# WeiZhang1988/YDORBSLAM

Hardware: AMD Instinct MI355X
Metric: ORB extract+match Mkeypoints/sec (higher is better)
Workload: dtype u8

## Files before the change

### ydorbslam_amd/csrc/extract_kernels.hip.h

```cpp
#pragma once
#include <hip/hip_runtime.h>
#include <stdint.h>

#include "quadtree_core.h"
#include "quadtree_flat.h"

#pragma clang fp contract(off)

namespace ydorb {

constexpr int kPad = 19;
constexpr int kBorder = 16;
constexpr int kMaxLevels = 8;
constexpr int kTileMax = 72;
#ifndef QT_THREADS
#define QT_THREADS 512
#endif
constexpr int kQtThreads = QT_THREADS;

struct LevelDev {
  int w, h, pitch;
  int padOff;
  int blurOff, blurPitch;
  int cellBegin, nCells;
  int quota;
  int candOff;
  int kpOff;
  int tabOff;
  int nodeTabOff;
  float scale;
  float size;
};
struct PlanDev {
  int nLevels, nCellsTotal, cellCap, sumQuota;
  int maxX[16];
  unsigned nodeTabFrameStride;
  int blurTileBegin[kMaxLevels + 1];
  int borderBegin[kMaxLevels + 1];
  LevelDev lv[kMaxLevels];
};
#ifndef BLUR_TH
#define BLUR_TH 58
#endif
constexpr int kBlurTW = 64, kBlurTH = BLUR_TH;
struct CellDev {
  short level, x0, y0, x1, y1, pad0;
  int srcOff;
};

__device__ __forceinline__ int reflect101(int i, int n) {
  if (n == 1) return 0;
  while (i < 0 || i >= n) i = i < 0 ? -i : 2 * (n - 1) - i;
  return i;
}

typedef uint32_t __attribute__((aligned(1))) u32_unaligned;
typedef unsigned long long __attribute__((aligned(1))) u64_unaligned;

#ifndef PYR_ROWS
#define PYR_ROWS 8
#endif
constexpr int kPyrRows = PYR_ROWS;
__global__ __launch_bounds__(256) void k_pyr_level0(const uint8_t* __restrict__ img, int stride, size_t frameStride,
                                                    uint8_t* __restrict__ pyr, size_t pyrFrameStride, LevelDev L) {
  const int wx = blockIdx.x * 64 + (threadIdx.x & 63);
  const int yb = (blockIdx.y * 4 + __builtin_amdgcn_readfirstlane(threadIdx.x >> 6)) * kPyrRows;
  const int x0 = wx * 4 - kPad;
  if (x0 + 3 < 0 || x0 >= L.w) return;
  const uint8_t* src = img + (size_t)blockIdx.z * frameStride;
  uint8_t* dst = pyr + (size_t)blockIdx.z * pyrFrameStride + L.padOff + (size_t)kPad * L.pitch + wx * 4;
  const int xa = L.w >= 4 ? min(max(x0, 0), L.w - 4) : 0, sh = 8 * (x0 - xa);
  uint32_t v[kPyrRows];
#pragma unroll
  for (int r = 0; r < kPyrRows; r++) {
    const uint8_t* row = src + (size_t)min(yb + r, L.h - 1) * stride;
    if (L.w >= 4) {
      v[r] = *reinterpret_cast<const u32_unaligned*>(row + xa);
    } else {
      v[r] = 0;
      for (int b = 0; b < L.w; b++) v[r] |= (uint32_t)row[b] << (8 * b);
    }
    v[r] = sh < 0 ? v[r] << (-sh) : v[r] >> sh;
  }
#pragma unroll
  for (int r = 0; r < kPyrRows; r++)
    if (yb + r < L.h) *reinterpret_cast<uint32_t*>(dst + (size_t)(yb + r) * L.pitch) = v[r];
}

__global__ __launch_bounds__(256) void k_pyr_resize(uint8_t* __restrict__ pyr, size_t pyrFrameStride, LevelDev Lp, LevelDev L,
                                                    double scaleX, const short* __restrict__ alpha,
                                                    const int* __restrict__ yofs, const short* __restrict__ beta) {
  const int wx = blockIdx.x * 64 + (threadIdx.x & 63);
  const int yb = (blockIdx.y * 4 + __builtin_amdgcn_readfirstlane(threadIdx.x >> 6)) * kPyrRows;
  const int x0 = wx * 4 - kPad;
  if (x0 + 3 < 0 || x0 >= L.w) return;
  uint8_t* frame = pyr + (size_t)blockIdx.z * pyrFrameStride;
  const uint8_t* S = frame + Lp.padOff + (size_t)kPad * Lp.pitch + kPad;
  uint8_t* dst = frame + L.padOff + (size_t)kPad * L.pitch + wx * 4;
  int sx[4], sx1[4], a0[4], a1[4];
#pragma unroll
  for (int b = 0; b < 4; b++) {
    const int dx = min(max(x0 + b, 0), L.w - 1);
    const float fx = (float)__dsub_rn(__dmul_rn((double)dx + 0.5, scaleX), 0.5);
    sx[b] = min(max((int)floorf(fx), 0), Lp.w - 1);
    a0[b] = alpha[2 * dx]; a1[b] = alpha[2 * dx + 1];
    sx1[b] = min(sx[b] + 1, Lp.w - 1);
  }
  const bool fast = sx[3] - sx[0] <= 6;
  const uint8_t *r0p[kPyrRows], *r1p[kPyrRows];
  int b0[kPyrRows], b1[kPyrRows];
#pragma unroll
  for (int r = 0; r < kPyrRows; r++) {
    const int dy = min(yb + r, L.h - 1);
    const int sy = yofs[dy];
    b0[r] = beta[2 * dy]; b1[r] = beta[2 * dy + 1];
    r0p[r] = S + (size_t)min(max(sy, 0), Lp.h - 1) * Lp.pitch;
    r1p[r] = S + (size_t)min(max(sy + 1, 0), Lp.h - 1) * Lp.pitch;
  }
// ... 1076 lines not shown
  const int c4 = (threadIdx.x & 15) * 4;
#pragma unroll
  for (int r = threadIdx.x >> 4; r < TH; r += 16) {
    const int gy = y0 + r;
    if (!(gy < L.h && x0 + c4 < L.blurPitch)) continue;
    typedef unsigned short u16x2 __attribute__((ext_vector_type(2)));
    const bool odd = r & 1;
    const u16x2 k0 = odd ? u16x2{0, 18} : u16x2{18, 34}, k1 = odd ? u16x2{34, 48} : u16x2{48, 56};
    const u16x2 k2 = odd ? u16x2{56, 48} : u16x2{48, 34}, k3 = odd ? u16x2{34, 18} : u16x2{18, 0};
    const uint32_t* hp = &hb[(r >> 1) * TW + c4];
    const uint4 p0 = *reinterpret_cast<const uint4*>(hp), p1 = *reinterpret_cast<const uint4*>(hp + TW);
    const uint4 p2 = *reinterpret_cast<const uint4*>(hp + 2 * TW), p3 = *reinterpret_cast<const uint4*>(hp + 3 * TW);
    const uint32_t q0[4] = {p0.x, p0.y, p0.z, p0.w}, q1[4] = {p1.x, p1.y, p1.z, p1.w}, q2[4] = {p2.x, p2.y, p2.z, p2.w}, q3[4] = {p3.x, p3.y, p3.z, p3.w};
    uint32_t acc[4];
#pragma unroll
    for (int k = 0; k < 4; k++) {
      acc[k] = __builtin_amdgcn_udot2(__builtin_bit_cast(u16x2, q0[k]), k0, 32768u, false);
      acc[k] = __builtin_amdgcn_udot2(__builtin_bit_cast(u16x2, q1[k]), k1, acc[k], false);
      acc[k] = __builtin_amdgcn_udot2(__builtin_bit_cast(u16x2, q2[k]), k2, acc[k], false);
      acc[k] = __builtin_amdgcn_udot2(__builtin_bit_cast(u16x2, q3[k]), k3, acc[k], false);
    }
    const uint32_t out = (acc[0] >> 16) | ((acc[1] >> 16) << 8) | ((acc[2] >> 16) << 16) | ((acc[3] >> 16) << 24);
    *reinterpret_cast<uint32_t*>(blur + (size_t)f * blurFrameStride + L.blurOff + (size_t)gy * L.blurPitch + x0 + c4) = out;
  }
}

__device__ __forceinline__ float fast_atan2_deg(float y, float x) {
  const float p1 = 0.9997878412794807f * (float)(180 / 3.14159265358979323846);
  const float p3 = -0.3258083974640975f * (float)(180 / 3.14159265358979323846);
  const float p5 = 0.1555786518463281f * (float)(180 / 3.14159265358979323846);
  const float p7 = -0.04432655554792128f * (float)(180 / 3.14159265358979323846);
  const float eps = (float)2.2204460492503131e-16;
  const float ax = fabsf(x), ay = fabsf(y);
  float a, c, c2;
  if (ax >= ay) {
    c = __fdiv_rn(ay, __fadd_rn(ax, eps));
    c2 = __fmul_rn(c, c);
    a = __fmul_rn(__fadd_rn(__fmul_rn(__fadd_rn(__fmul_rn(__fadd_rn(__fmul_rn(p7, c2), p5), c2), p3), c2), p1), c);
  } else {
    c = __fdiv_rn(ax, __fadd_rn(ay, eps));
    c2 = __fmul_rn(c, c);
    a = __fsub_rn(90.f, __fmul_rn(__fadd_rn(__fmul_rn(__fadd_rn(__fmul_rn(__fadd_rn(__fmul_rn(p7, c2), p5), c2), p3), c2), p1), c));
  }
  if (x < 0) a = __fsub_rn(180.f, a);
  if (y < 0) a = __fsub_rn(360.f, a);
  return a;
}

__device__ __forceinline__ void sincos_det(float xf, float* sinOut, float* cosOut) {
  const double x = (double)xf;
  const double n = rint(__dmul_rn(x, 6.36619772367581382433e-01));
  const double r = __dsub_rn(__dsub_rn(x, __dmul_rn(n, 1.57079632673412561417e+00)), __dmul_rn(n, 6.07710050650619224932e-11));
  const double z = __dmul_rn(r, r);
  double p = __dmul_rn(z, 1.58969099521155010221e-10);
  p = __dadd_rn(p, -2.50507602534068634195e-08); p = __dmul_rn(p, z);
  p = __dadd_rn(p, 2.75573137070700676789e-06);  p = __dmul_rn(p, z);
  p = __dadd_rn(p, -1.98412698298579493134e-04); p = __dmul_rn(p, z);
  p = __dadd_rn(p, 8.33333333332248946124e-03);  p = __dmul_rn(p, z);
  p = __dadd_rn(p, -1.66666666666666324348e-01); p = __dmul_rn(p, z);
  p = __dmul_rn(p, r); p = __dadd_rn(p, r);
  double q = __dmul_rn(z, -1.13596475577881948265e-11);
  q = __dadd_rn(q, 2.08757232129817482790e-09);  q = __dmul_rn(q, z);
  q = __dadd_rn(q, -2.75573143513906633035e-07); q = __dmul_rn(q, z);
  q = __dadd_rn(q, 2.48015872894767294178e-05);  q = __dmul_rn(q, z);
  q = __dadd_rn(q, -1.38888888888741095749e-03); q = __dmul_rn(q, z);
  q = __dadd_rn(q, 4.16666666666666019037e-02);  q = __dmul_rn(q, z);
  q = __dmul_rn(q, z);
  double h = __dmul_rn(z, 0.5);
  h = __dsub_rn(h, q);
  h = __dsub_rn(1.0, h);
  const int quad = ((int)n) & 3;
  const double sv = quad == 0 ? p : quad == 1 ? h : quad == 2 ? -p : -h;
  const double cv = quad == 0 ? h : quad == 1 ? -p : quad == 2 ? -h : p;
  *sinOut = (float)sv;
  *cosOut = (float)cv;
}

__device__ __align__(16) const float kPatternDev[1024] = {
#include "orb_pattern_data.inc"
};

struct YdKeyPointDev { float x, y, size, angle, response; int octave, class_id; };

__global__ __launch_bounds__(256) void k_orient_describe(const uint8_t* __restrict__ pyr, size_t pyrFrameStride,
                                                         const uint8_t* __restrict__ blur, size_t blurFrameStride, PlanDev P,
                                                         const uint32_t* __restrict__ lvlKp, const int* __restrict__ lvlCount,
                                                         YdKeyPointDev* __restrict__ kps, uint8_t* __restrict__ desc, int cap,
                                                         int* __restrict__ nOut, float* __restrict__ lvlAngle) {
  const int lane = threadIdx.x & 63;
  int bx = blockIdx.x, f = blockIdx.y;
  if ((f | 7) < (int)gridDim.y) {
    bx = (f & 7) * (gridDim.x >> 3) + (blockIdx.x >> 3);
    f = (f & ~7) | (blockIdx.x & 7);
  }
  const int slot = bx * 4 + __builtin_amdgcn_readfirstlane(threadIdx.x >> 6);
  if (slot >= P.sumQuota) return;
  float4 pat[4];
#pragma unroll
  for (int t = 0; t < 4; t++) pat[t] = reinterpret_cast<const float4*>(kPatternDev)[t * 64 + lane];
  int level = 0;
#pragma unroll
  for (int l = 1; l < kMaxLevels; l++)
    if (l < P.nLevels && slot >= P.lv[l].kpOff) level = l;
  const uint32_t pk = __builtin_amdgcn_readfirstlane(lvlKp[(size_t)f * P.sumQuota + slot]);
  int before = 0, tot = 0, mine = 0;
#pragma unroll
  for (int l = 0; l < kMaxLevels; l++) {
    const int c = l < P.nLevels ? lvlCount[f * kMaxLevels + l] : 0;
    if (l < level) before += c;
    if (l == level) mine = c;
    tot += c;
  }
  if (slot == 0 && lane == 0) nOut[f] = min(tot, cap);
  const LevelDev L = P.lv[level];
  const int k = slot - L.kpOff;
  if (k >= mine) return;
  const int outIdx = before + k;
  if (outIdx >= cap) return;
  const int kx = qt_x(pk) + kBorder, ky = qt_y(pk) + kBorder;
  const uint8_t* roi = pyr + (size_t)f * pyrFrameStride + L.padOff + (size_t)kPad * L.pitch + kPad;
  const uint8_t* org = roi + (ptrdiff_t)(ky - 15) * L.pitch + (kx - 32);
  const int u = lane - 32;
  unsigned narrow = 0;
#pragma unroll
  for (int v = 1; v <= 15; v++) narrow |= (unsigned)(P.maxX[v] == 0) << v;
  int m10 = 0, m01 = 0;
  if (u >= -15 && u <= 15) m10 = u * org[(unsigned)(15 * L.pitch + lane)];
  if (lane >= 1 && lane <= 15 && ((narrow >> lane) & 1u)) {
    const int pos = org[(unsigned)((15 + lane) * L.pitch + 32)], neg = org[(unsigned)((15 - lane) * L.pitch + 32)];
    m01 = lane * (pos - neg);
  }
#pragma unroll
  for (int v = 1; v <= 15; v++) {
    const int d = P.maxX[v];
    if (d > 0 && u >= -d && u <= d) {
      const int pos = org[(unsigned)((15 + v) * L.pitch + lane)], neg = org[(unsigned)((15 - v) * L.pitch + lane)];
      m01 += v * (pos - neg);
      m10 += u * (pos + neg);
    }
  }
#pragma unroll
  for (int o = 32; o >= 1; o >>= 1) {
    m10 += __shfl_xor(m10, o, 64);
    m01 += __shfl_xor(m01, o, 64);
  }
  const float angle = fast_atan2_deg((float)m01, (float)m10);
  const float rad = __fmul_rn(angle, (float)(3.14159265358979323846 / 180.0));
  float sinB, cosA;
  sincos_det(rad, &sinB, &cosA);
  constexpr int kBias = 24;
  const uint8_t* bl = blur + (size_t)f * blurFrameStride + L.blurOff + (ptrdiff_t)(ky - kBias) * L.blurPitch + (kx - kBias);
  unsigned long long words[4];
#pragma unroll
  for (int t = 0; t < 4; t++) {
    const float4 pt = pat[t];
    const int r0 = __float2int_rn(__fadd_rn(__fmul_rn(pt.x, sinB), __fmul_rn(pt.y, cosA)));
    const int c0 = __float2int_rn(__fsub_rn(__fmul_rn(pt.x, cosA), __fmul_rn(pt.y, sinB)));
    const int r1 = __float2int_rn(__fadd_rn(__fmul_rn(pt.z, sinB), __fmul_rn(pt.w, cosA)));
    const int c1 = __float2int_rn(__fsub_rn(__fmul_rn(pt.z, cosA), __fmul_rn(pt.w, sinB)));
    const int t0 = bl[(unsigned)((r0 + kBias) * L.blurPitch + c0 + kBias)], t1 = bl[(unsigned)((r1 + kBias) * L.blurPitch + c1 + kBias)];
    words[t] = __ballot(t0 < t1);
  }
  if (lane < 4) {
    unsigned long long w = lane == 0 ? words[0] : lane == 1 ? words[1] : lane == 2 ? words[2] : words[3];
    reinterpret_cast<unsigned long long*>(desc + ((size_t)f * cap + outIdx) * 32)[lane] = w;
  }
  if (lane == 0) {
    YdKeyPointDev kp;
    kp.x = (float)kx;
    kp.y = (float)ky;
    if (level) { kp.x = __fmul_rn(kp.x, L.scale); kp.y = __fmul_rn(kp.y, L.scale); }
    kp.size = L.size;
    kp.angle = angle;
    kp.response = (float)qt_r(pk);
    kp.octave = level;
    kp.class_id = -1;
    kps[(size_t)f * cap + outIdx] = kp;
    lvlAngle[(size_t)f * P.sumQuota + slot] = angle;
  }
}


template <int KPW>
__global__ __launch_bounds__(256) void k_orient_describe_n(const uint8_t* __restrict__ pyr, size_t pyrFrameStride,
                                                           const uint8_t* __restrict__ blur, size_t blurFrameStride, PlanDev P,
                                                           const uint32_t* __restrict__ lvlKp, const int* __restrict__ lvlCount,
                                                           YdKeyPointDev* __restrict__ kps, uint8_t* __restrict__ desc, int cap,
                                                           int* __restrict__ nOut, float* __restrict__ lvlAngle) {
  const int lane = threadIdx.x & 63;
  int bx = blockIdx.x, f = blockIdx.y;
  if ((f | 7) < (int)gridDim.y) {
    bx = (f & 7) * (gridDim.x >> 3) + (blockIdx.x >> 3);
    f = (f & ~7) | (blockIdx.x & 7);
  }
  const int slot0 = (bx * 4 + __builtin_amdgcn_readfirstlane(threadIdx.x >> 6)) * KPW;
  if (slot0 >= P.sumQuota) return;
  float4 pat[4];
#pragma unroll
  for (int t = 0; t < 4; t++) pat[t] = reinterpret_cast<const float4*>(kPatternDev)[t * 64 + lane];
  int cnt[kMaxLevels], tot = 0;
#pragma unroll
  for (int l = 0; l < kMaxLevels; l++) { cnt[l] = l < P.nLevels ? lvlCount[f * kMaxLevels + l] : 0; tot += cnt[l]; }
  int level[KPW], outIdx[KPW];
  uint32_t pk[KPW];
  bool valid[KPW];
#pragma unroll
  for (int j = 0; j < KPW; j++) {
    const int slot = min(slot0 + j, P.sumQuota - 1);
    level[j] = 0;
#pragma unroll
    for (int l = 1; l < kMaxLevels; l++)
      if (l < P.nLevels && slot >= P.lv[l].kpOff) level[j] = l;
    pk[j] = __builtin_amdgcn_readfirstlane(lvlKp[(size_t)f * P.sumQuota + slot]);
  }
  if (slot0 == 0 && lane == 0) nOut[f] = min(tot, cap);
  bool any = false;
#pragma unroll
  for (int j = 0; j < KPW; j++) {
    int before = 0, mine = 0;
#pragma unroll
    for (int l = 0; l < kMaxLevels; l++) {
      if (l < level[j]) before += cnt[l];
      if (l == level[j]) mine = cnt[l];
    }
    const int k = slot0 + j - P.lv[level[j]].kpOff;
    outIdx[j] = before + k;
    valid[j] = slot0 + j < P.sumQuota && k < mine && outIdx[j] < cap;
    any = any || valid[j];
  }
  if (!any) return;
  int firstValid = 0;
#pragma unroll
  for (int j = KPW - 1; j >= 0; j--) if (valid[j]) firstValid = j;
#pragma unroll
  for (int j = 0; j < KPW; j++)
    if (!valid[j]) {
#pragma unroll
      for (int i = 0; i < KPW; i++) if (i == firstValid) { pk[j] = pk[i]; level[j] = level[i]; }
    }
  int kx[KPW], ky[KPW], pitch[KPW];
  const uint8_t* org[KPW];
#pragma unroll
  for (int j = 0; j < KPW; j++) {
    const LevelDev& L = P.lv[level[j]];
    kx[j] = qt_x(pk[j]) + kBorder; ky[j] = qt_y(pk[j]) + kBorder;
    pitch[j] = L.pitch;
    const uint8_t* roi = pyr + (size_t)f * pyrFrameStride + L.padOff + (size_t)kPad * L.pitch + kPad;
    org[j] = roi + (ptrdiff_t)(ky[j] - 15) * L.pitch + (kx[j] - 32);
  }
  const int u = lane - 32;
  unsigned narrow = 0;
#pragma unroll
  for (int v = 1; v <= 15; v++) narrow |= (unsigned)(P.maxX[v] == 0) << v;
  int m10[KPW], m01[KPW];
#pragma unroll
  for (int j = 0; j < KPW; j++) {
    m10[j] = 0; m01[j] = 0;
    if (u >= -15 && u <= 15) m10[j] = u * org[j][(unsigned)(15 * pitch[j] + lane)];
    if (lane >= 1 && lane <= 15 && ((narrow >> lane) & 1u)) {
      const int pos = org[j][(unsigned)((15 + lane) * pitch[j] + 32)], neg = org[j][(unsigned)((15 - lane) * pitch[j] + 32)];
      m01[j] = lane * (pos - neg);
    }
  }
#pragma unroll
  for (int v = 1; v <= 15; v++) {
    const int d = P.maxX[v];
    if (d > 0 && u >= -d && u <= d) {
#pragma unroll
      for (int j = 0; j < KPW; j++) {
        const int pos = org[j][(unsigned)((15 + v) * pitch[j] + lane)], neg = org[j][(unsigned)((15 - v) * pitch[j] + lane)];
        m01[j] += v * (pos - neg);
        m10[j] += u * (pos + neg);
      }
    }
  }
#pragma unroll
  for (int o = 32; o >= 1; o >>= 1) {
#pragma unroll
    for (int j = 0; j < KPW; j++) {
      m10[j] += __shfl_xor(m10[j], o, 64);
      m01[j] += __shfl_xor(m01[j], o, 64);
    }
  }
  constexpr int kBias = 24;
  float angle[KPW];
  int tA[KPW][4], tB[KPW][4];
#pragma unroll
  for (int j = 0; j < KPW; j++) {
    const LevelDev& L = P.lv[level[j]];
    angle[j] = fast_atan2_deg((float)m01[j], (float)m10[j]);
    const float rad = __fmul_rn(angle[j], (float)(3.14159265358979323846 / 180.0));
    float sinB, cosA;
    sincos_det(rad, &sinB, &cosA);
    const uint8_t* bl = blur + (size_t)f * blurFrameStride + L.blurOff + (ptrdiff_t)(ky[j] - kBias) * L.blurPitch + (kx[j] - kBias);
#pragma unroll
    for (int t = 0; t < 4; t++) {
      const float4 pt = pat[t];
      const int r0 = __float2int_rn(__fadd_rn(__fmul_rn(pt.x, sinB), __fmul_rn(pt.y, cosA)));
      const int c0 = __float2int_rn(__fsub_rn(__fmul_rn(pt.x, cosA), __fmul_rn(pt.y, sinB)));
      const int r1 = __float2int_rn(__fadd_rn(__fmul_rn(pt.z, sinB), __fmul_rn(pt.w, cosA)));
      const int c1 = __float2int_rn(__fsub_rn(__fmul_rn(pt.z, cosA), __fmul_rn(pt.w, sinB)));
      tA[j][t] = bl[(unsigned)((r0 + kBias) * L.blurPitch + c0 + kBias)];
      tB[j][t] = bl[(unsigned)((r1 + kBias) * L.blurPitch + c1 + kBias)];
    }
  }
#pragma unroll
  for (int j = 0; j < KPW; j++) {
    unsigned long long words[4];
#pragma unroll
    for (int t = 0; t < 4; t++) words[t] = __ballot(tA[j][t] < tB[j][t]);
    if (!valid[j]) continue;
    const LevelDev& L = P.lv[level[j]];
    if (lane < 4) {
      unsigned long long w = lane == 0 ? words[0] : lane == 1 ? words[1] : lane == 2 ? words[2] : words[3];
      reinterpret_cast<unsigned long long*>(desc + ((size_t)f * cap + outIdx[j]) * 32)[lane] = w;
    }
    if (lane == 0) {
      YdKeyPointDev kp;
      kp.x = (float)kx[j];
      kp.y = (float)ky[j];
      if (level[j]) { kp.x = __fmul_rn(kp.x, L.scale); kp.y = __fmul_rn(kp.y, L.scale); }
      kp.size = L.size;
      kp.angle = angle[j];
      kp.response = (float)qt_r(pk[j]);
      kp.octave = level[j];
      kp.class_id = -1;
      kps[(size_t)f * cap + outIdx[j]] = kp;
      lvlAngle[(size_t)f * P.sumQuota + slot0 + j] = angle[j];
    }
  }
}

}
```

### ydorbslam_amd/csrc/orb_extractor.hip

```cpp
#include <hip/hip_runtime.h>
#include <cstdlib>

#include <algorithm>
#include <cmath>
#include <cstdarg>
#include <cstdio>
#include <cstring>
#include <string>
#include <vector>

#include "../../include/ydorb/c_api.h"
#include "extract_kernels.hip.h"
#include "host_buffers.h"
#include "ydorb_host.h"

using namespace ydorb;

namespace {

inline int cvRoundF(float v) { return (int)lrintf(v); }
inline int cvFloorF(float v) { int i = (int)v; return i - (i > v); }
inline int alignUp(int v, int a) { return (v + a - 1) / a * a; }
inline size_t alignUpZ(size_t v, size_t a) { return (v + a - 1) / a * a; }

// ... 92 lines not shown

void buildFusedLevel(HostPlan& P, int l) {
  const PlanDev& D = P.dev;
  const LevelDev& L = D.lv[l];
  HostPlan::FusedLevel& F = P.fused[l];
  F.on = false;
  if (L.w < 20 || L.h < 20) return;
  const int nd = (L.w + 2 * kPad + 3) >> 2;
  auto srcOf = [&](int p) { return p < kPad ? 2 * kPad - p : p < kPad + L.w ? -1 : p < L.w + 2 * kPad ? 2 * L.w + 2 * kPad - 2 - p : -2; };
  int shift = -1;
  for (int sft = 0; sft < 64 && shift < 0; sft++) {
    bool ok = true;
    for (int c = 0; c < nd && ok; c++)
      for (int j = 0; j < 4; j++) {
        const int sp = srcOf(4 * c + j);
        if (sp >= 0 && ((sp >> 2) + sft) >> 6 != (c + sft) >> 6) ok = false;
      }
    if (ok) shift = sft;
  }
  if (shift < 0) return;
  std::vector<PyrColEntry> col;
  if (l > 0) {
    const LevelDev& Lp = D.lv[l - 1];
    const int* xofs = P.tabInt.data() + P.tab[l].xofs;
    const short* alpha = P.tabShort.data() + P.tab[l].alpha;
    col.resize(nd);
    for (int c = 0; c < nd; c++) {
      const int dx0 = std::min(std::max(4 * c - kPad, 0), L.w - 1);
      for (int b = 0; b < 4; b++) {
        const int dx = std::min(std::max(4 * c - kPad + b, 0), L.w - 1);
        const int off = xofs[dx] - xofs[dx0];
        if (off < 0 || off > 6 || xofs[dx0] + 7 >= Lp.w + kPad) return;
        col[c].sel[b] = (uint32_t)off | 0x0c000c00u | ((uint32_t)(off + 1) << 16);
        col[c].ab[b] = (uint32_t)(uint16_t)alpha[2 * dx] | ((uint32_t)(uint16_t)alpha[2 * dx + 1] << 16);
      }
    }
  }
  F.shift = shift;
  F.padOff = (int)P.padTab.size();
  for (int c = 0; c < nd; c++) {
    int dA = -1, dB = -1;
    for (int j = 0; j < 4; j++) {
      const int sp = srcOf(4 * c + j);
      if (sp < 0) continue;
      const int d = sp >> 2;
      if (dA < 0 || d == dA) dA = d;
      else dB = d;
    }
    PyrPadEntry pe{};
    pe.laneA4 = 4u * (unsigned)(((dA < 0 ? c : dA) + shift) & 63);
    pe.laneB4 = 4u * (unsigned)(((dB < 0 ? c : dB) + shift) & 63);
    pe.selM = 0; pe.selF = 0;
    for (int j = 0; j < 4; j++) {
      const int sp = srcOf(4 * c + j);
      uint32_t m = 0x0c, f;
      if (sp == -1) f = (uint32_t)j;
      else if (sp == -2) f = 0x0c;
      else { m = (uint32_t)(sp & 3) + ((sp >> 2) == dA ? 4u : 0u); f = 4u + (uint32_t)j; }
      pe.selM |= m << (8 * j);
      pe.selF |= f << (8 * j);
    }
    P.padTab.push_back(pe);
  }
  if (l > 0) {
    F.colOff = (int)P.colTab.size();
    P.colTab.insert(P.colTab.end(), col.begin(), col.end());
    F.rowOff = (int)P.rowTab.size();
    const int* yofs = P.tabInt.data() + P.tab[l].yofs;
    const short* beta = P.tabShort.data() + P.tab[l].beta;
    const int rows = alignUp(L.h, 4 * kPyrRowsF);
    for (int y = 0; y < rows; y++) {
      const int dy = std::min(y, L.h - 1);
      P.rowTab.push_back(make_int2(yofs[dy], (int)((uint32_t)(uint16_t)beta[2 * dy] | ((uint32_t)(uint16_t)beta[2 * dy + 1] << 16))));
    }
  }
  F.on = true;
}

int buildPlan(ydorb_extractor* e, int w, int h, HostPlan& P) {
  P = HostPlan();
  P.w = w; P.h = h;
  PlanDev& D = P.dev;
  D.nLevels = e->cfg.n_levels;
  for (int v = 0; v < 16; v++) D.maxX[v] = e->maxX[v];
  size_t padOff = 0, blurOff = 0;
  int kpOff = 0, candOff = 0, maxCellDim = 0;
  for (int l = 0; l < D.nLevels; l++) {
    LevelDev& L = D.lv[l];
    L.w = cvRoundF((float)w * e->isf[l]);
    L.h = cvRoundF((float)h * e->isf[l]);
    if (L.w < 1 || L.h < 1 || L.w > 4000 || L.h > 4000) {
      set_error("level %d size %dx%d out of the supported range (1..4000)", l, L.w, L.h);
      return YDORB_ERR_UNSUPPORTED;
    }
    L.pitch = alignUp(L.w + 2 * kPad, 64);
    L.padOff = (int)padOff;
    padOff += alignUpZ((size_t)(L.h + 2 * kPad) * L.pitch, 256);
    L.blurPitch = alignUp(L.w, 64);
    L.blurOff = (int)blurOff;
    blurOff += alignUpZ((size_t)L.h * L.blurPitch, 256);
    L.quota = e->perLevel[l];
    L.kpOff = kpOff;
    kpOff += L.quota;
    L.scale = e->sf[l];
    L.size = (float)(int)(31 * e->sf[l]);
    L.cellBegin = (int)P.cells.size();
    const int minB = kBorder, maxBX = L.w - kBorder, maxBY = L.h - kBorder;
    const float width = (float)(maxBX - minB), height = (float)(maxBY - minB);
    const int colsNum = (int)(width / 30.0f), rowsNum = (int)(height / 30.0f);
    if (colsNum > 0 && rowsNum > 0) {
      const int cellW = (int)ceilf(width / colsNum), cellH = (int)ceilf(height / rowsNum);
      maxCellDim = std::max(maxCellDim, std::max(cellW, cellH));
      P.levelCellDim[l] = std::max(cellW, cellH);
      for (int i = 0; i < rowsNum; i++) {
        const float iniY = (float)(minB + i * cellH);
        float maxY = iniY + cellH + 6;
        if (iniY >= maxBY - 3) continue;
        if (maxY > maxBY) maxY = (float)maxBY;
        for (int j = 0; j < colsNum; j++) {
          const float iniX = (float)(minB + j * cellW);
          float maxX = iniX + cellW + 6;
          if (iniX >= maxBX - 6) continue;
          if (maxX > maxBX) maxX = (float)maxBX;
          CellDev c{};
          c.level = (short)l;
          c.x0 = (short)iniX; c.y0 = (short)iniY; c.x1 = (short)maxX; c.y1 = (short)maxY;
          c.srcOff = L.padOff + (kPad + c.y0) * L.pitch + kPad + c.x0;
          P.cells.push_back(c);
        }
      }
    }
    L.nCells = (int)P.cells.size() - L.cellBegin;
    if (l > 0) {
      const LevelDev& Lp = D.lv[l - 1];
      const double scale_x = 1. / ((double)L.w / Lp.w), scale_y = 1. / ((double)L.h / Lp.h);
      P.tab[l].xofs = (int)P.tabInt.size();
      P.tab[l].alpha = (int)P.tabShort.size();
      for (int dx = 0; dx < L.w; dx++) {
        float fx = (float)((dx + 0.5) * scale_x - 0.5);
        int sx = cvFloorF(fx);
        fx -= sx;
        if (sx < 0) { fx = 0; sx = 0; }
        if (sx >= Lp.w - 1) { fx = 0; sx = Lp.w - 1; }
        P.tabInt.push_back(sx);
        P.tabShort.push_back((short)cvRoundF((1.f - fx) * 2048));
        P.tabShort.push_back((short)cvRoundF(fx * 2048));
      }
      P.tab[l].yofs = (int)P.tabInt.size();
      P.tab[l].beta = (int)P.tabShort.size();
      for (int dy = 0; dy < L.h; dy++) {
        float fy = (float)((dy + 0.5) * scale_y - 0.5);
        int sy = cvFloorF(fy);
        fy -= sy;
        P.tabInt.push_back(sy);
        P.tabShort.push_back((short)cvRoundF((1.f - fy) * 2048));
        P.tabShort.push_back((short)cvRoundF(fy * 2048));
      }
    }
  }
  if (maxCellDim + 6 > kTileMax) {
    set_error("cell size %d exceeds the FAST tile (%d)", maxCellDim, kTileMax - 6);
    return YDORB_ERR_UNSUPPORTED;
  }
  D.nCellsTotal = (int)P.cells.size();
  P.maxCellDim = maxCellDim;
  D.cellCap = alignUp(std::max(((maxCellDim + 1) / 2) * ((maxCellDim + 1) / 2), 64), 64);
  D.sumQuota = kpOff;
// ... 178 lines not shown
      const int maxT = dim + 6, maxB = dim;
      narrow = maxT <= 44;
      const int pitch = narrow ? 48 : 80;
      fl.tileBytes = alignUp((maxT + 3) * pitch, 16);
      fl.scoreBytes = alignUp((maxB + 2) * (maxB + 2) + 4, 16);
      fl.listBytes = alignUp(2 * maxB * maxB, 16);
      return (size_t)4 * (fl.tileBytes + fl.scoreBytes + fl.listBytes);
    };
    {
      FastLds flAll; bool nAll;
      const size_t dynAll = fastGeom(0, D.nLevels, flAll, nAll);
      if (dynAll > 48 * 1024) {
        HIPCHK(hipFuncSetAttribute(reinterpret_cast<const void*>(k_fast_cells<48>), hipFuncAttributeMaxDynamicSharedMemorySize, (int)dynAll));
        HIPCHK(hipFuncSetAttribute(reinterpret_cast<const void*>(k_fast_cells<80>), hipFuncAttributeMaxDynamicSharedMemorySize, (int)dynAll));
      }
    }
    int l0 = 0;
    for (int g = 0; g < e->fastGroups && l0 < D.nLevels; g++) {
      const int l1 = g == e->fastGroups - 1 ? D.nLevels : l0 + 1;
      const int c0 = D.lv[l0].cellBegin, c1 = D.lv[l1 - 1].cellBegin + D.lv[l1 - 1].nCells;
      if (c1 > c0 && D.nCellsTotal > 0) {
        FastLds fl; bool narrow;
        const size_t dyn = fastGeom(l0, l1, fl, narrow);
        const dim3 grid(((c1 - c0 + 3) / 4 + 7) / 8 * 8, nFrames);
        if (narrow) hipLaunchKernelGGL(k_fast_cells<48>, grid, dim3(256), dyn, s, e->d_pyr, P.pyrFrameStride, D, e->d_cells, c0, c1, thr, fl, e->d_cellCount, e->d_cellCand);
        else hipLaunchKernelGGL(k_fast_cells<80>, grid, dim3(256), dyn, s, e->d_pyr, P.pyrFrameStride, D, e->d_cells, c0, c1, thr, fl, e->d_cellCount, e->d_cellCand);
      }
      HIPCHK(hipEventRecord(e->evFast[l0], s));
      fastEv[l0] = e->evFast[l0];
      grpFirst[nGroups] = l0; grpEnd[nGroups] = l1; nGroups++;
      for (int l = l0 + 1; l < l1; l++) fastEv[l] = e->evFast[l0];
      l0 = l1;
    }
  }
  if (prof) HIPCHK(hipEventRecord(e->ev[2], s));
  HIPCHK(hipEventRecord(e->evFork, s));
  hipLaunchKernelGGL(k_blur, dim3((D.blurTileBegin[D.nLevels] + 7) / 8 * 8, nFrames), dim3(256), 0, s, e->d_pyr, P.pyrFrameStride, e->d_blur,
                     P.blurFrameStride, D);
  if (prof) HIPCHK(hipEventRecord(e->ev[3], s));
  bool anyFast = false;
  for (int g = 0; g < nGroups; g++) {
    const int l0 = grpFirst[g], l1 = grpEnd[g];
    const hipStream_t qs = e->qtInline ? s : e->qtStream[g % kMaxLevels];
    if (!e->qtInline) HIPCHK(hipStreamWaitEvent(qs, fastEv[l0] ? fastEv[l0] : e->evFork, 0));
    int items = 8, qmax = 1, tabLen = 2;
    for (int l = l0; l < l1; l++) {
      items = std::max(items, P.qt[l].items); qmax = std::max(qmax, D.lv[l].quota);
      tabLen = std::max(tabLen, std::max(D.lv[l].w - 2 * kBorder, 0) + std::max(D.lv[l].h - 2 * kBorder, 0) + 2);
    }
    const size_t lds = qt_fast_lds_bytes(qmax, tabLen);
    if (!e->forcePassQuadtree && lds <= 150 * 1024) {
      const dim3 grid(nFrames, l1 - l0);
#define YD_QT_FAST(IT) hipLaunchKernelGGL(k_qt_fast<IT>, grid, dim3(kQfThreads), lds, qs, D, e->d_cellCount, e->d_cellCand, l0, qmax, tabLen, e->d_lvlKp, \
                                          e->d_lvlCount, e->d_needPass, e->d_lvlMaxN, e->d_passList, e->d_passList + 1)
      if (items <= 8) YD_QT_FAST(8);
      else if (items <= 16) YD_QT_FAST(16);
      else YD_QT_FAST(32);
#undef YD_QT_FAST
      anyFast = true;
    } else {
      for (int l = l0; l < l1; l++) {
        const HostPlan::QtLevel& Q = P.qt[l];
        hipLaunchKernelGGL(k_quadtree, dim3(1, nFrames), dim3(kQtThreads), Q.lds, qs, D, e->d_cellCount, e->d_cellCand, e->d_qtCand, e->d_qtNode,
                           P.qtFrameStride, Q.nodeCap, Q.candCap, l, e->d_lvlKp, e->d_lvlCount, e->d_status, e->d_nodeScratch);
      }
    }
    if (!e->qtInline) HIPCHK(hipEventRecord(e->evJoin[g], qs));
  }
  if (!e->qtInline) for (int g = 0; g < nGroups; g++) HIPCHK(hipStreamWaitEvent(s, e->evJoin[g], 0));
  if (anyFast) {
    const int seen = e->h_lvlMaxN[kMaxLevels];
    const int listGrid = std::max(1, std::min({kQtPassWorkgroups, D.nLevels * nFrames, seen + seen / 4}));
    hipLaunchKernelGGL(k_quadtree_list, dim3(listGrid), dim3(kQtListThreads), P.qtPassLds, s, D, e->d_cellCount, e->d_cellCand,
                       e->d_qtCand, e->d_qtNode, P.qtFrameStride, -std::max(P.qtPassNodes, 1), e->d_lvlKp, e->d_lvlCount, e->d_status, e->d_passList,
                       e->d_passList + 1, e->d_nodeScratch, e->d_lvlMaxN + kMaxLevels);
    HIPCHK(hipMemsetAsync(e->d_passList, 0, sizeof(int), s));
  }
  if (prof) HIPCHK(hipEventRecord(e->ev[4], s));
  {
    const int kpw = e->descKpw;
    const dim3 gd(((D.sumQuota + 4 * kpw - 1) / (4 * kpw) + 7) / 8 * 8, nFrames);
#define YD_DESC(K) hipLaunchKernelGGL((k_orient_describe_n<K>), gd, dim3(256), 0, s, e->d_pyr, P.pyrFrameStride, e->d_blur, P.blurFrameStride, D, \
                                         e->d_lvlKp, e->d_lvlCount, d_kps, d_desc, cap, d_nOut, e->d_lvlAngle)
    if (kpw == 1)
      hipLaunchKernelGGL(k_orient_describe, gd, dim3(256), 0, s, e->d_pyr, P.pyrFrameStride, e->d_blur,
                         P.blurFrameStride, D, e->d_lvlKp, e->d_lvlCount, d_kps, d_desc, cap, d_nOut, e->d_lvlAngle);
    else if (kpw == 2) YD_DESC(2);
    else YD_DESC(4);
#undef YD_DESC
  }
  if (prof) { HIPCHK(hipEventRecord(e->ev[5], s)); e->profPending = true; }
  HIPCHK(hipMemcpyAsync(e->h_lvlMaxN, e->d_lvlMaxN, sizeof(int) * (kMaxLevels + 1), hipMemcpyDeviceToHost, s));
  HIPCHK(hipGetLastError());
  e->lastFrames = nFrames;
  e->lastStream = s;
  return YDORB_OK;
}

int checkStatus(ydorb_extractor* e) {
  if (*e->h_status == 1) { set_error("more than 65535 FAST candidates in one pyramid level"); return YDORB_ERR_CAPACITY; }
  if (*e->h_status == 3) { set_error("a pyramid level needs the pass quad-tree kernel (more candidates than LDS slots, or a very deep tree) but its quota is too large for that kernel's LDS node table"); return YDORB_ERR_CAPACITY; }
  if (*e->h_status) { set_error("quad-tree node table overflow (status %d)", *e->h_status); return YDORB_ERR_CAPACITY; }
  return YDORB_OK;
}

void collectProfile(ydorb_extractor* e) {
  if (!e->profiling || !e->profPending) return;
  e->profPending = false;
  for (int i = 0; i < ST_COUNT; i++) {
    float ms = 0;
    if (hipEventElapsedTime(&ms, e->ev[i], e->ev[i + 1]) == hipSuccess) e->stageMs[i] += ms;
  }
  e->stageCalls++;
}

}

int ydorb::extractor_pyramid_view(const ydorb_extractor* e, PyramidView* v) {
  if (!e || !v || !e->planValid || e->lastFrames < 1) { set_error("the extractor holds no pyramid (no call yet)"); return YDORB_ERR_INVALID_ARG; }
  v->device = e->cfg.device; v->nLevels = e->cfg.n_levels; v->frames = e->lastFrames; v->frameStride = (long long)e->plan.pyrFrameStride;
  v->stream = e->stream;
  for (int l = 0; l < e->cfg.n_levels; l++) {
    const LevelDev& L = e->plan.dev.lv[l];
    v->roi[l] = e->d_pyr + L.padOff + (size_t)kPad * L.pitch + kPad;
    v->w[l] = L.w; v->h[l] = L.h; v->pitch[l] = L.pitch;
    v->scale[l] = e->sf[l]; v->invScale[l] = e->isf[l];
    v->quota[l] = e->perLevel[l];
  }
  return YDORB_OK;
}

extern "C" {

int ydorb_extractor_create(const YdExtractorConfig* cfg, ydorb_extractor_t** out) {
  if (!cfg || !out) { set_error("null argument"); return YDORB_ERR_INVALID_ARG; }
  *out = nullptr;
  if (cfg->n_levels < 1 || cfg->n_levels > kMaxLevels || cfg->n_features < 1 || !(cfg->scale_factor > 1.0f)) {
    set_error("unsupported extractor config (n_levels 1..8, n_features >= 1, scale_factor > 1)");
    return YDORB_ERR_INVALID_ARG;
  }
  int rc = ydorb::require_device(cfg->device);
  if (rc) return rc;
  ydorb_extractor* e = new ydorb_extractor();
  e->cfg = *cfg;
  if (const char* v = getenv("YDORB_QT_PASS")) e->forcePassQuadtree = v[0] == '1';
  if (const char* v = getenv("YDORB_PYR_FUSED")) e->noFusedPads = v[0] == '0';
  e->descKpw = cfg->max_batch <= 8 ? 1 : 4;
  if (const char* v = getenv("YDORB_DESC_KPW")) e->descKpw = atoi(v) == 1 ? 1 : atoi(v) == 4 ? 4 : 2;
  e->cfg.min_fast_thr = cfg->ini_fast_thr;
  const int L = cfg->n_levels;
  const float s = cfg->scale_factor;
  int per = (int)round(cfg->n_features * (1 - 1.0 / s) / (1.0 - pow(1.0 / s, L)));
  int sum = 0;
  for (int i = 0; i < L; i++) {
    e->sf.push_back((float)pow(s, i));
    e->sf2.push_back((float)pow(s, 2 * i));
    e->isf.push_back((float)pow(s, -i));
    e->isf2.push_back((float)pow(s, -2 * i));
    if (i < L - 1) {
      e->perLevel.push_back(per);
      sum += per;
      per = (int)round((float)per / s);
    } else {
      e->perLevel.push_back(std::max(cfg->n_features - sum, 0));
    }
  }
  e->sumQuota = 0;
  for (int q : e->perLevel) e->sumQuota += q;
  {
    const int half = 15;
    std::vector<int> mx(half + 1, 0);
    const int maxY = (int)floor(half * sqrt(2.0) / 2.0 + 1.0), minY = (int)ceil(half * sqrt(2.0) / 2.0);
    for (int v = 0; v <= maxY; v++) mx.push_back((int)round(sqrt((double)half * half + (double)v * v)));
    for (int v = half, i = 0; v >= minY; v--) {
      while (mx[i] == mx[i + 1]) i++;
      mx[v] = i;
      i++;
    }
    for (int v = 0; v < 16; v++) e->maxX[v] = mx[v];
  }
  if (hipStreamCreateWithFlags(&e->stream, hipStreamNonBlocking) != hipSuccess) {
    set_error("hipStreamCreate failed");
    delete e;
    return YDORB_ERR_HIP;
  }
  for (auto& ev : e->ev) (void)hipEventCreate(&ev);
  (void)hipEventCreateWithFlags(&e->evFork, hipEventDisableTiming);
  for (int l = 0; l < kMaxLevels; l++) {
    const char* qtEnv = getenv("YDORB_QT_STREAMS");
    e->qtInline = (qtEnv && atoi(qtEnv) == 0) || (cfg->flags & YDORB_EXTRACTOR_SINGLE_STREAM);
    const int nQt = std::max(1, std::min(qtEnv ? atoi(qtEnv) : (cfg->max_batch <= 8 ? (int)kMaxLevels : 2), (int)kMaxLevels));
    if (l < nQt) (void)hipStreamCreateWithFlags(&e->qtStream[l], hipStreamNonBlocking);
    else e->qtStream[l] = e->qtStream[l % nQt];
    (void)hipEventCreateWithFlags(&e->evJoin[l], hipEventDisableTiming);
    (void)hipEventCreateWithFlags(&e->evFast[l], hipEventDisableTiming);
  }
  {
    const char* g = getenv("YDORB_FAST_GROUPS");
    e->fastGroups = std::max(1, std::min(g ? atoi(g) : (cfg->max_batch <= 8 ? 1 : 2), (int)kMaxLevels));
  }
  *out = e;
  return YDORB_OK;
}

void ydorb_extractor_destroy(ydorb_extractor_t* e) {
  if (!e) return;
  (void)hipSetDevice(e->cfg.device);
  if (e->stream) (void)hipStreamSynchronize(e->stream);
  freeBuffers(e);
  for (auto& ev : e->ev) if (ev) (void)hipEventDestroy(ev);
  for (int l = 0; l < kMaxLevels; l++) {
    if (e->qtStream[l]) {
      bool shared = false;
      for (int k = 0; k < l; k++) shared = shared || e->qtStream[k] == e->qtStream[l];
      if (!shared) { (void)hipStreamSynchronize(e->qtStream[l]); (void)hipStreamDestroy(e->qtStream[l]); }
    }
    if (e->evJoin[l]) (void)hipEventDestroy(e->evJoin[l]);
    if (e->evFast[l]) (void)hipEventDestroy(e->evFast[l]);
  }
  if (e->evFork) (void)hipEventDestroy(e->evFork);
  if (e->stream) (void)hipStreamDestroy(e->stream);
  delete e;
}

int ydorb_extractor_tables(const ydorb_extractor_t* e, float* scale, float* inv_scale, float* scale_sq, float* inv_scale_sq,
                           int32_t* per_level) {
  if (!e) { set_error("null handle"); return YDORB_ERR_INVALID_ARG; }
  for (int i = 0; i < e->cfg.n_levels; i++) {
    if (scale) scale[i] = e->sf[i];
    if (inv_scale) inv_scale[i] = e->isf[i];
    if (scale_sq) scale_sq[i] = e->sf2[i];
    if (inv_scale_sq) inv_scale_sq[i] = e->isf2[i];
    if (per_level) per_level[i] = e->perLevel[i];
  }
  return YDORB_OK;
}

int ydorb_extractor_max_keypoints(const ydorb_extractor_t* e) { return e ? e->sumQuota : YDORB_ERR_INVALID_ARG; }

int ydorb_extract_batch_device(ydorb_extractor_t* e, const uint8_t* d_img, int32_t w, int32_t h, int32_t stride, size_t frame_stride,
                               int32_t n_frames, YdKeyPoint* d_kps, uint8_t* d_desc, int32_t cap, int32_t* d_n_out, void* stream) {
  if (!e || !d_img || !d_kps || !d_desc || !d_n_out || w <= 0 || h <= 0 || n_frames <= 0 || stride < w) {
    set_error("invalid argument");
    return YDORB_ERR_INVALID_ARG;
  }
  if (cap < e->sumQuota) { set_error("cap %d < max keypoints %d", cap, e->sumQuota); return YDORB_ERR_CAPACITY; }
  HIPCHK(hipSetDevice(e->cfg.device));
  int rc = ensurePlan(e, w, h, n_frames);
  if (rc) return rc;
  return enqueue(e, d_img, stride, frame_stride, n_frames, reinterpret_cast<YdKeyPointDev*>(d_kps), d_desc, cap, d_n_out,
                 stream ? (hipStream_t)stream : e->stream);
}

int ydorb_extractor_synchronize(ydorb_extractor_t* e) {
  if (!e) { set_error("null handle"); return YDORB_ERR_INVALID_ARG; }
  HIPCHK(hipSetDevice(e->cfg.device));
  HIPCHK(hipStreamSynchronize(e->stream));
  if (e->lastStream && e->lastStream != e->stream) HIPCHK(hipStreamSynchronize(e->lastStream));
  if (!e->d_status) return YDORB_OK;
  HIPCHK(hipMemcpy(e->h_status, e->d_status, sizeof(int), hipMemcpyDeviceToHost));
  const int rc = checkStatus(e);
  if (rc) HIPCHK(hipMemset(e->d_status, 0, sizeof(int)));
  return rc;
// ... 193 lines not shown
```

Measured before the change: 182.5.

## Compile-time orientation circle table, fold narrow rows into half-waves, share atan per lane

Replaces the runtime maxX table in PlanDev with a constexpr table so the per-row loop bounds are known at compile time. Rows whose half-width is at most 15 are repacked so each half of the wave handles one of the +v/-v rows, halving loads for those rows. The centre row and the narrow-column pixels are merged into a single load per lane. atan2 and sincos are computed once per keypoint on separate lanes and broadcast with readlane, instead of every lane computing them for all KPW keypoints. The single-keypoint kernel is dropped in favour of the template with KPW=1, and a host check rejects configurations whose table differs from the constant.

```diff
diff --git a/ydorbslam_amd/csrc/extract_kernels.hip.h b/ydorbslam_amd/csrc/extract_kernels.hip.h
--- a/ydorbslam_amd/csrc/extract_kernels.hip.h
+++ b/ydorbslam_amd/csrc/extract_kernels.hip.h
@@ -33,7 +33,6 @@
 };
 struct PlanDev {
   int nLevels, nCellsTotal, cellCap, sumQuota;
-  int maxX[16];
   unsigned nodeTabFrameStride;
   int blurTileBegin[kMaxLevels + 1];
   int borderBegin[kMaxLevels + 1];
@@ -1276,104 +1275,7 @@
 
 struct YdKeyPointDev { float x, y, size, angle, response; int octave, class_id; };
 
-__global__ __launch_bounds__(256) void k_orient_describe(const uint8_t* __restrict__ pyr, size_t pyrFrameStride,
-                                                         const uint8_t* __restrict__ blur, size_t blurFrameStride, PlanDev P,
-                                                         const uint32_t* __restrict__ lvlKp, const int* __restrict__ lvlCount,
-                                                         YdKeyPointDev* __restrict__ kps, uint8_t* __restrict__ desc, int cap,
-                                                         int* __restrict__ nOut, float* __restrict__ lvlAngle) {
-  const int lane = threadIdx.x & 63;
-  int bx = blockIdx.x, f = blockIdx.y;
-  if ((f | 7) < (int)gridDim.y) {
-    bx = (f & 7) * (gridDim.x >> 3) + (blockIdx.x >> 3);
-    f = (f & ~7) | (blockIdx.x & 7);
-  }
-  const int slot = bx * 4 + __builtin_amdgcn_readfirstlane(threadIdx.x >> 6);
-  if (slot >= P.sumQuota) return;
-  float4 pat[4];
-#pragma unroll
-  for (int t = 0; t < 4; t++) pat[t] = reinterpret_cast<const float4*>(kPatternDev)[t * 64 + lane];
-  int level = 0;
-#pragma unroll
-  for (int l = 1; l < kMaxLevels; l++)
-    if (l < P.nLevels && slot >= P.lv[l].kpOff) level = l;
-  const uint32_t pk = __builtin_amdgcn_readfirstlane(lvlKp[(size_t)f * P.sumQuota + slot]);
-  int before = 0, tot = 0, mine = 0;
-#pragma unroll
-  for (int l = 0; l < kMaxLevels; l++) {
-    const int c = l < P.nLevels ? lvlCount[f * kMaxLevels + l] : 0;
-    if (l < level) before += c;
-    if (l == level) mine = c;
-    tot += c;
-  }
-  if (slot == 0 && lane == 0) nOut[f] = min(tot, cap);
-  const LevelDev L = P.lv[level];
-  const int k = slot - L.kpOff;
-  if (k >= mine) return;
-  const int outIdx = before + k;
-  if (outIdx >= cap) return;
-  const int kx = qt_x(pk) + kBorder, ky = qt_y(pk) + kBorder;
-  const uint8_t* roi = pyr + (size_t)f * pyrFrameStride + L.padOff + (size_t)kPad * L.pitch + kPad;
-  const uint8_t* org = roi + (ptrdiff_t)(ky - 15) * L.pitch + (kx - 32);
-  const int u = lane - 32;
-  unsigned narrow = 0;
-#pragma unroll
-  for (int v = 1; v <= 15; v++) narrow |= (unsigned)(P.maxX[v] == 0) << v;
-  int m10 = 0, m01 = 0;
-  if (u >= -15 && u <= 15) m10 = u * org[(unsigned)(15 * L.pitch + lane)];
-  if (lane >= 1 && lane <= 15 && ((narrow >> lane) & 1u)) {
-    const int pos = org[(unsigned)((15 + lane) * L.pitch + 32)], neg = org[(unsigned)((15 - lane) * L.pitch + 32)];
-    m01 = lane * (pos - neg);
-  }
-#pragma unroll
-  for (int v = 1; v <= 15; v++) {
-    const int d = P.maxX[v];
-    if (d > 0 && u >= -d && u <= d) {
-      const int pos = org[(unsigned)((15 + v) * L.pitch + lane)], neg = org[(unsigned)((15 - v) * L.pitch + lane)];
-      m01 += v * (pos - neg);
-      m10 += u * (pos + neg);
-    }
-  }
-#pragma unroll
-  for (int o = 32; o >= 1; o >>= 1) {
-    m10 += __shfl_xor(m10, o, 64);
-    m01 += __shfl_xor(m01, o, 64);
-  }
-  const float angle = fast_atan2_deg((float)m01, (float)m10);
-  const float rad = __fmul_rn(angle, (float)(3.14159265358979323846 / 180.0));
-  float sinB, cosA;
-  sincos_det(rad, &sinB, &cosA);
-  constexpr int kBias = 24;
-  const uint8_t* bl = blur + (size_t)f * blurFrameStride + L.blurOff + (ptrdiff_t)(ky - kBias) * L.blurPitch + (kx - kBias);
-  unsigned long long words[4];
-#pragma unroll
-  for (int t = 0; t < 4; t++) {
-    const float4 pt = pat[t];
-    const int r0 = __float2int_rn(__fadd_rn(__fmul_rn(pt.x, sinB), __fmul_rn(pt.y, cosA)));
-    const int c0 = __float2int_rn(__fsub_rn(__fmul_rn(pt.x, cosA), __fmul_rn(pt.y, sinB)));
-    const int r1 = __float2int_rn(__fadd_rn(__fmul_rn(pt.z, sinB), __fmul_rn(pt.w, cosA)));
-    const int c1 = __float2int_rn(__fsub_rn(__fmul_rn(pt.z, cosA), __fmul_rn(pt.w, sinB)));
-    const int t0 = bl[(unsigned)((r0 + kBias) * L.blurPitch + c0 + kBias)], t1 = bl[(unsigned)((r1 + kBias) * L.blurPitch + c1 + kBias)];
-    words[t] = __ballot(t0 < t1);
-  }
-  if (lane < 4) {
-    unsigned long long w = lane == 0 ? words[0] : lane == 1 ? words[1] : lane == 2 ? words[2] : words[3];
-    reinterpret_cast<unsigned long long*>(desc + ((size_t)f * cap + outIdx) * 32)[lane] = w;
-  }
-  if (lane == 0) {
-    YdKeyPointDev kp;
-    kp.x = (float)kx;
-    kp.y = (float)ky;
-    if (level) { kp.x = __fmul_rn(kp.x, L.scale); kp.y = __fmul_rn(kp.y, L.scale); }
-    kp.size = L.size;
-    kp.angle = angle;
-    kp.response = (float)qt_r(pk);
-    kp.octave = level;
-    kp.class_id = -1;
-    kps[(size_t)f * cap + outIdx] = kp;
-    lvlAngle[(size_t)f * P.sumQuota + slot] = angle;
-  }
-}
-
+constexpr int kOrientMaxX[16] = {0, 0, 0, 0, 0, 0, 0, 0, 0, 0, 0, 26, 25, 22, 19, 15};
 
 template <int KPW>
 __global__ __launch_bounds__(256) void k_orient_describe_n(const uint8_t* __restrict__ pyr, size_t pyrFrameStride,
@@ -1442,29 +1344,46 @@
     const uint8_t* roi = pyr + (size_t)f * pyrFrameStride + L.padOff + (size_t)kPad * L.pitch + kPad;
     org[j] = roi + (ptrdiff_t)(ky[j] - 15) * L.pitch + (kx[j] - 32);
   }
-  const int u = lane - 32;
+  const int u = lane - 32, hl = lane & 31, uh = hl - 15;
+  const bool upper = lane >= 32;
   unsigned narrow = 0;
 #pragma unroll
-  for (int v = 1; v <= 15; v++) narrow |= (unsigned)(P.maxX[v] == 0) << v;
+  for (int v = 1; v <= 15; v++) narrow |= (unsigned)(kOrientMaxX[v] == 0) << v;
+  const int nv = (hl >> 1) + 1, nsv = (hl & 1) ? -nv : nv;
+  const bool actA = upper ? (hl < 30 && ((narrow >> nv) & 1u)) : hl < 31;
+  const int rowA = upper ? 15 + nsv : 15, colA = upper ? 32 : 17 + hl;
+  const int wA10 = upper ? 0 : uh, wA01 = upper ? nsv : 0;
   int m10[KPW], m01[KPW];
 #pragma unroll
   for (int j = 0; j < KPW; j++) {
     m10[j] = 0; m01[j] = 0;
-    if (u >= -15 && u <= 15) m10[j] = u * org[j][(unsigned)(15 * pitch[j] + lane)];
-    if (lane >= 1 && lane <= 15 && ((narrow >> lane) & 1u)) {
-      const int pos = org[j][(unsigned)((15 + lane) * pitch[j] + 32)], neg = org[j][(unsigned)((15 - lane) * pitch[j] + 32)];
-      m01[j] = lane * (pos - neg);
+    if (actA) {
+      const int pix = org[j][(unsigned)(rowA * pitch[j] + colA)];
+      m10[j] = wA10 * pix;
+      m01[j] = wA01 * pix;
     }
   }
 #pragma unroll
   for (int v = 1; v <= 15; v++) {
-    const int d = P.maxX[v];
-    if (d > 0 && u >= -d && u <= d) {
-#pragma unroll
-      for (int j = 0; j < KPW; j++) {
-        const int pos = org[j][(unsigned)((15 + v) * pitch[j] + lane)], neg = org[j][(unsigned)((15 - v) * pitch[j] + lane)];
-        m01[j] += v * (pos - neg);
-        m10[j] += u * (pos + neg);
+    const int d = kOrientMaxX[v];
+    if (d > 15) {
+      if (u >= -d && u <= d) {
+#pragma unroll
+        for (int j = 0; j < KPW; j++) {
+          const int pos = org[j][(unsigned)((15 + v) * pitch[j] + lane)], neg = org[j][(unsigned)((15 - v) * pitch[j] + lane)];
+          m01[j] += v * (pos - neg);
+          m10[j] += u * (pos + neg);
+        }
+      }
+    } else if (d > 0) {
+      if (uh >= -d && uh <= d) {
+        const int row = upper ? 15 - v : 15 + v, sv = upper ? -v : v;
+#pragma unroll
+        for (int j = 0; j < KPW; j++) {
+          const int pix = org[j][(unsigned)(row * pitch[j] + 17 + hl)];
+          m01[j] += sv * pix;
+          m10[j] += uh * pix;
+        }
       }
     }
   }
@@ -1476,16 +1395,22 @@
       m01[j] += __shfl_xor(m01[j], o, 64);
     }
   }
+  int my01 = m01[0], my10 = m10[0];
+#pragma unroll
+  for (int j = 1; j < KPW; j++)
+    if (lane == j) { my01 = m01[j]; my10 = m10[j]; }
+  const float myAngle = fast_atan2_deg((float)my01, (float)my10);
+  float mySin, myCos;
+  sincos_det(__fmul_rn(myAngle, (float)(3.14159265358979323846 / 180.0)), &mySin, &myCos);
   constexpr int kBias = 24;
   float angle[KPW];
   int tA[KPW][4], tB[KPW][4];
 #pragma unroll
   for (int j = 0; j < KPW; j++) {
     const LevelDev& L = P.lv[level[j]];
-    angle[j] = fast_atan2_deg((float)m01[j], (float)m10[j]);
-    const float rad = __fmul_rn(angle[j], (float)(3.14159265358979323846 / 180.0));
-    float sinB, cosA;
-    sincos_det(rad, &sinB, &cosA);
+    angle[j] = __builtin_bit_cast(float, __builtin_amdgcn_readlane(__builtin_bit_cast(int, myAngle), j));
+    const float sinB = __builtin_bit_cast(float, __builtin_amdgcn_readlane(__builtin_bit_cast(int, mySin), j));
+    const float cosA = __builtin_bit_cast(float, __builtin_amdgcn_readlane(__builtin_bit_cast(int, myCos), j));
     const uint8_t* bl = blur + (size_t)f * blurFrameStride + L.blurOff + (ptrdiff_t)(ky[j] - kBias) * L.blurPitch + (kx[j] - kBias);
 #pragma unroll
     for (int t = 0; t < 4; t++) {
diff --git a/ydorbslam_amd/csrc/orb_extractor.hip b/ydorbslam_amd/csrc/orb_extractor.hip
--- a/ydorbslam_amd/csrc/orb_extractor.hip
+++ b/ydorbslam_amd/csrc/orb_extractor.hip
@@ -198,7 +198,6 @@
   P.w = w; P.h = h;
   PlanDev& D = P.dev;
   D.nLevels = e->cfg.n_levels;
-  for (int v = 0; v < 16; v++) D.maxX[v] = e->maxX[v];
   size_t padOff = 0, blurOff = 0;
   int kpOff = 0, candOff = 0, maxCellDim = 0;
   for (int l = 0; l < D.nLevels; l++) {
@@ -543,9 +542,7 @@
     const dim3 gd(((D.sumQuota + 4 * kpw - 1) / (4 * kpw) + 7) / 8 * 8, nFrames);
 #define YD_DESC(K) hipLaunchKernelGGL((k_orient_describe_n<K>), gd, dim3(256), 0, s, e->d_pyr, P.pyrFrameStride, e->d_blur, P.blurFrameStride, D, \
                                          e->d_lvlKp, e->d_lvlCount, d_kps, d_desc, cap, d_nOut, e->d_lvlAngle)
-    if (kpw == 1)
-      hipLaunchKernelGGL(k_orient_describe, gd, dim3(256), 0, s, e->d_pyr, P.pyrFrameStride, e->d_blur,
-                         P.blurFrameStride, D, e->d_lvlKp, e->d_lvlCount, d_kps, d_desc, cap, d_nOut, e->d_lvlAngle);
+    if (kpw == 1) YD_DESC(1);
     else if (kpw == 2) YD_DESC(2);
     else YD_DESC(4);
 #undef YD_DESC
@@ -640,6 +637,12 @@
     }
     for (int v = 0; v < 16; v++) e->maxX[v] = mx[v];
   }
+  for (int v = 0; v < 16; v++)
+    if (e->maxX[v] != kOrientMaxX[v]) {
+      set_error("orientation row table differs from the kernel's constant at row %d", v);
+      delete e;
+      return YDORB_ERR_INVALID_ARG;
+    }
   if (hipStreamCreateWithFlags(&e->stream, hipStreamNonBlocking) != hipSuccess) {
     set_error("hipStreamCreate failed");
     delete e;
```

Result: no change. 182.0 (-0.3%).
